# DonsetPG/graph-physics

Hardware: AMD Instinct MI355X
Metric: training steps/sec, CylinderFlow 15-round MGN (batch 16 meshes per step) (higher is better)
Workload: dtype f32; 1 GPU; BASELINE.json configs[1], fp32: 16 x 1885-node CylinderFlow-like meshes per GPU (N=30160, E=180082), 15 rounds, latent 128, random init; global_batch_meshes=16, launch=eager, parallelism=single

## Files before the change

### graph-physics_amd/csrc/mgn_kernels.hip

```cpp
#include <hip/hip_runtime.h>
#include <stdint.h>
#include <stdlib.h>
#include <type_traits>
#include "mgn_hip.h"

typedef float f32x4 __attribute__((ext_vector_type(4)));

#define MFMA16(a, b, c) __builtin_amdgcn_mfma_f32_16x16x4f32((a), (b), (c), 0, 0, 0)

typedef __attribute__((address_space(1))) const f32x4 g_cf32x4;
typedef __attribute__((address_space(1))) f32x4 g_f32x4;
typedef __attribute__((address_space(1))) const float g_cfloat;
typedef __attribute__((address_space(1))) float g_float;
__device__ __forceinline__ f32x4 ld4(const float* p) { return *(g_cf32x4*)p; }
__device__ __forceinline__ void st4(float* p, f32x4 v) { *(g_f32x4*)p = v; }
__device__ __forceinline__ void st4_stream(float* p, f32x4 v) { *(g_f32x4*)p = v; }
__device__ __forceinline__ float ld1(const float* p) { return *(g_cfloat*)p; }
__device__ __forceinline__ void st1(float* p, float v) { *(g_float*)p = v; }

template <int HB, int MT>
__device__ __forceinline__ void gemm_tl(f32x4 (&acc)[MT][HB], const f32x4 (&in)[MT][HB],
                                        const float* __restrict__ W, int ldw, int nib, int nkb,
                                        int c, int g) {
  const float* wl = W + (size_t)c * ldw + 4 * g;
  constexpr int IP = (HB >= 2) ? 2 : 1;
#pragma unroll
  for (int ib = 0; ib < HB; ib += IP) {
    if (ib < nib) {
#pragma unroll
      for (int kb = 0; kb < HB; ++kb) {
        if (kb < nkb) {
          f32x4 w[IP];
#pragma unroll
          for (int q = 0; q < IP; ++q)
            w[q] = (ib + q < nib) ? ld4(wl + (size_t)(16 * (ib + q)) * ldw + 16 * kb) : f32x4{0.f, 0.f, 0.f, 0.f};
#pragma unroll
          for (int r = 0; r < 4; ++r)
#pragma unroll
            for (int t = 0; t < MT; ++t)
#pragma unroll
              for (int q = 0; q < IP; ++q)
                acc[t][ib + q] = MFMA16(w[q][r], in[t][kb][r], acc[t][ib + q]);
        }
      }
    }
  }
}

template <int HB, int MT, bool NEXT>
__device__ __forceinline__ void gemm_full(f32x4 (&acc)[MT][HB], f32x4 (&in)[MT][HB],
                                          const float* __restrict__ W, int ldw, int c, int g,
                                          const float* const (&nxt)[MT]) {
  constexpr int IP = (HB >= 2) ? 2 : 1;
  constexpr int NI = HB / IP;
  constexpr int NS = HB * NI;
// ... 1295 lines not shown
    const unsigned nb0 = sm0 + (buf ^ 1) * 2 * WG_TILE_BYTES;
    lds_char* ta = sm + buf * 2 * WG_TILE_BYTES;
    lds_char* tb = ta + WG_TILE_BYTES;
    const bool tail = (tile + 1) * WG_TILE_ROWS > J.M;
    float av[2][8], bv[2][2];
    ld_quad(ta, tb, 0, av[0], bv[0]);
    const int rows_left = (int)(J.M - tile * WG_TILE_ROWS);
    auto body = [&](auto TAIL) {
#pragma unroll
      for (int quad = 0; quad < WG_TILE_ROWS / 4; ++quad) {
        if (quad + 1 < WG_TILE_ROWS / 4) ld_quad(ta, tb, quad + 1, av[(quad + 1) & 1], bv[(quad + 1) & 1]);
        if (more && quad < 4) {
          dma_row_piece(J.A, (tile + 1) * WG_TILE_ROWS, J.M, nb0, wv, lane, quad);
          dma_row_piece(J.B, (tile + 1) * WG_TILE_ROWS, J.M, nb0 + WG_TILE_BYTES, wv, lane, quad);
        }
        __builtin_amdgcn_sched_barrier(0);
        if (decltype(TAIL)::value) {
          const float keep = (4 * quad + g < rows_left) ? 1.f : 0.f;
#pragma unroll
          for (int jb = 0; jb < 8; ++jb) av[quad & 1][jb] *= keep;
        }
#pragma unroll
        for (int kk = 0; kk < 2; ++kk)
#pragma unroll
          for (int jb = 0; jb < 8; ++jb) acc[kk][jb] = MFMA16(av[quad & 1][jb], bv[quad & 1][kk], acc[kk][jb]);
        if (want_db) {
#pragma unroll
          for (int jb = 0; jb < 8; ++jb) cs[jb] += av[quad & 1][jb];
        }
        __builtin_amdgcn_sched_barrier(0);
      }
    };
    if (tail)
      body(std::true_type{});
    else
      body(std::false_type{});
    TL_STAMP(7);
  }
  TL_DUMP();
  float* P = L.partial + (size_t)blockIdx.x * (128 * 128 + 128);
  if (want_db) {
#pragma unroll
    for (int jb = 0; jb < 8; ++jb) {
      const float v = rowsum4(cs[jb]);
      if (g == 0) P[128 * 128 + 16 * jb + c] = v;
    }
  }
#pragma unroll
  for (int kk = 0; kk < 2; ++kk)
#pragma unroll
    for (int jb = 0; jb < 8; ++jb)
#pragma unroll
      for (int q = 0; q < 4; ++q) P[(16 * jb + 4 * g + q) * 128 + 16 * (kb0 + kk) + c] = acc[kk][jb][q];
}

#include "mgn_x6.inc"
#include "mgn_pp.inc"
#include "mgn_ppr.inc"
#include "mgn_fused.inc"

template <bool BF, bool A16 = false, bool B16 = false>
__global__ void __launch_bounds__(256, 2) k_wgrad_row64(const WgradLaunch L) {
  constexpr int H = 64;
  __shared__ float red[3][H * H + H];
  const int lane = threadIdx.x & 63, wv = threadIdx.x >> 6;
  const int c = lane & 15, g = lane >> 4;
  int j, wg, nwg;
  wgrad_where(L, j, wg, nwg);
  const mgn_wgrad_job J = L.job[j];
  const int pidx = L.wg0[j] + wg;
  const long ntiles = (J.M + 15) >> 4;
  const long t0 = ntiles * wg / nwg, t1 = ntiles * (wg + 1) / nwg;
  const bool a_on = 4 * c < 16 * J.nja, b_on = 4 * c < J.kw;

  f32x4 acc[4][4];
#pragma unroll
  for (int qa = 0; qa < 4; ++qa)
#pragma unroll
    for (int qb = 0; qb < 4; ++qb) acc[qa][qb] = f32x4{0.f, 0.f, 0.f, 0.f};
  f32x4 cs = {0.f, 0.f, 0.f, 0.f};
  const f32x4 zero = {0.f, 0.f, 0.f, 0.f};
  f32x4 av[2][4], bv[2][4];
  constexpr bool a16 = BF && A16, b16 = BF && B16;
  const long plda = A16 ? -(long)J.lda : J.lda, pldb = B16 ? -(long)J.ldb : J.ldb;
  auto ld16 = [&](const float* X, long off) -> f32x4 {
    const uint2 t = *(const uint2*)((const uint16_t*)X + off);
    return f32x4{__uint_as_float(t.x << 16), __uint_as_float(t.x & 0xffff0000u), __uint_as_float(t.y << 16), __uint_as_float(t.y & 0xffff0000u)};
  };
  auto load_tile = [&](long tile, f32x4 (&a)[4], f32x4 (&b)[4]) {
#pragma unroll
    for (int r = 0; r < 4; ++r) {
      const long row = tile * 16 + 4 * g + r;
      const bool ok = row < J.M;
      if constexpr (a16) a[r] = (ok && a_on) ? ld16(J.A, row * plda + 4 * c) : zero;
      else a[r] = (ok && a_on) ? ld4(J.A + row * plda + 4 * c) : zero;
      if constexpr (b16) b[r] = (ok && b_on) ? ld16(J.B, row * pldb + 4 * c) : zero;
      else b[r] = (ok && b_on) ? ld4(J.B + row * pldb + 4 * c) : zero;
    }
  };
  auto mac_tile = [&](const f32x4 (&a)[4], const f32x4 (&b)[4]) {
    if constexpr (BF) {
      typedef short s16x4 __attribute__((ext_vector_type(4)));
      typedef u32 u32x2_ __attribute__((ext_vector_type(2)));
      s16x4 pa[4], pb[4];
#pragma unroll
      for (int q = 0; q < 4; ++q) {
// ... 1104 lines not shown
    case 128: lrc = launch_bwd<8>(a, s); break;
    case 64: lrc = launch_bwd<4>(a, s); break;
    case 32: lrc = launch_bwd<2>(a, s); break;
    default: lrc = launch_bwd<1>(a, s); break;
  }
  if (lrc) return fail(2, "mgn_mlp_bwd: cannot reserve LDS");
  if (int rc = check_launch("mgn_mlp_bwd")) return rc;
  const unsigned grid = plan_mlp(a.M, a.H, a.NL, a.out_w != a.H || a.n_din > 1, true, a.act).grid;
  const int nslot = a.NL + 1;
  ColredOuts outs;
  bool any = false;
  for (int l = 0; l <= MGN_MAX_LAYERS; ++l) outs.o[l] = nullptr;
  for (int l = 0; l < a.NL; ++l) {
    outs.o[l] = a.db[l];
    any |= a.db[l] != nullptr;
  }
  outs.o[a.NL] = (a.scale != nullptr) ? a.dscale : nullptr;
  any |= outs.o[a.NL] != nullptr;
  if (!any || a.defer_reduce) return 0;
  const int n = nslot * a.H;
  hipLaunchKernelGGL(k_colred, dim3((n + 31) / 32), dim3(1024), 0, s, (const float*)a.red_ws, (int)grid, nslot, a.H, outs);
  return check_launch("mgn_mlp_bwd/colred");
}

int mgn_colred_batch(int n, const mgn_colred_job* jobs, void* stream) {
  if (n < 0) return fail(1, "mgn_colred_batch: bad arguments");
  hipStream_t s = (hipStream_t)stream;
  for (int i0 = 0; i0 < n; i0 += CR_MAX) {
    ColredBatch B;
    const int m = (n - i0 < CR_MAX) ? n - i0 : CR_MAX;
    int maxcol = 0;
    for (int i = 0; i < m; ++i) {
      const mgn_colred_job& q = jobs[i0 + i];
      if (q.red_ws == nullptr || q.NL < 1 || q.NL > MGN_MAX_LAYERS) return fail(1, "mgn_colred_batch: bad job");
      ColredJob& J = B.j[i];
      J.ws = (const float*)q.red_ws;
      J.nblocks = (int)plan_mlp(q.M, q.H, q.NL, q.out_w != q.H || q.n_din > 1, true).grid;
      J.nslot = q.NL + 1;
      J.H = q.H;
      for (int l = 0; l <= MGN_MAX_LAYERS; ++l) J.outs.o[l] = nullptr;
      for (int l = 0; l < q.NL; ++l) J.outs.o[l] = q.db[l];
      J.outs.o[q.NL] = q.dscale;
      if (J.nslot * J.H > maxcol) maxcol = J.nslot * J.H;
    }
    hipLaunchKernelGGL(k_colred_batch, dim3((maxcol + 31) / 32, m), dim3(1024), 0, s, B);
  }
  return check_launch("mgn_colred_batch");
}

static bool wgrad_job_row64(const mgn_wgrad_job& j) {
  return j.nja <= 4 && j.nkb <= 4 && j.kw <= 64 && (j.kw & 3) == 0 && (j.lda & 3) == 0 && (j.ldb & 3) == 0 &&
         (((uintptr_t)j.A | (uintptr_t)j.B) & 15) == 0;
}
static int wgrad_plan(int njobs, const mgn_wgrad_job* jobs, int* wg0, bool lds, int lds_budget = 512) {
  const int rows = lds ? WG_TILE_ROWS : 16;
  int budget = lds ? lds_budget : 512;
  if (!lds) {
    if (const char* e = getenv("MGN_WGRAD_GENERIC_BUDGET")) {
      const int b = atoi(e);
      if (b >= 64 && b <= 1024) budget = b;
    }
  }
  int64_t tiles[MGN_MAX_WGRAD_JOBS], tot = 0;
  int n[MGN_MAX_WGRAD_JOBS];
  for (int j = 0; j < njobs; ++j) {
    tiles[j] = (jobs[j].M + rows - 1) / rows;
    if (tiles[j] < 1) tiles[j] = 1;
    tot += tiles[j];
  }
  int used = 0;
  for (int j = 0; j < njobs; ++j) {
    int64_t s = tiles[j] * budget / tot;
    const int64_t cap = (tiles[j] + 3) / 4;
    if (s > cap) s = cap;
    if (s < 1) s = 1;
    n[j] = (int)s;
    used += n[j];
  }
  while (used < budget) {
    int best = -1;
    double load = 4.0;
    for (int j = 0; j < njobs; ++j) {
      const double l = (double)tiles[j] / n[j];
      if (l > load) {
        load = l;
        best = j;
      }
    }
    if (best < 0) break;
    ++n[best];
    ++used;
  }
  int acc = 0;
  for (int j = 0; j < njobs; ++j) {
    wg0[j] = acc;
    acc += n[j];
  }
  wg0[njobs] = acc;
  return acc;
}

size_t mgn_wgrad_workspace_bytes(int njobs, const mgn_wgrad_job* jobs) {
  if (njobs < 1 || njobs > MGN_MAX_WGRAD_JOBS) return 0;
  return (size_t)(512 + 1024 + 2 * MGN_MAX_WGRAD_JOBS) * (128 * 128 + 128) * sizeof(float);
}

static bool wgrad_job_full(const mgn_wgrad_job& j) {
  return j.nja == 8 && j.nkb == 8 && (j.lda == 128 || j.lda == -128) && (j.ldb == 128 || j.ldb == -128) && j.kw == 128 && j.M >= 1 && getenv("MGN_NO_LDS") == nullptr;
}

int mgn_wgrad(int njobs, const mgn_wgrad_job* jobs, void* ws, size_t ws_bytes, void* stream) {
  return mgn_wgrad_p(njobs, jobs, ws, ws_bytes, 0, stream);
}

int mgn_wgrad_p(int njobs, const mgn_wgrad_job* jobs, void* ws, size_t ws_bytes, int precision, void* stream) {
  if (precision != 0 && precision != 1) return fail(1, "mgn_wgrad: precision must be 0 (fp32-grade) or 1 (bf16)");
  if (njobs < 1 || njobs > MGN_MAX_WGRAD_JOBS) return fail(1, "mgn_wgrad: njobs out of range");
  for (int j = 0; j < njobs; ++j) {
    if (jobs[j].lda < 0 || jobs[j].ldb < 0) {
      const bool r64 = !wgrad_job_full(jobs[j]) && wgrad_job_row64(jobs[j]) && getenv("MGN_WGRAD_NO_ROW64") == nullptr &&
                       ((((uintptr_t)jobs[j].A | (uintptr_t)jobs[j].B) & 15) == 0);
      if (precision != 1 || !(wgrad_job_full(jobs[j]) || r64) || getenv("MGN_FP32_MFMA") != nullptr)
        return fail(1, "mgn_wgrad: a negative leading dimension (bf16 rows) needs precision 1 and a full 128 x 128 job with ld = -128 or a job of the row-vector kernel");
    }
  }
  hipStream_t s = (hipStream_t)stream;
  size_t ws_off = 0;
  for (int pass = 0; pass < 2; ++pass) {
    WgradLaunch L;
    L.njobs = 0;
    int maxb = 1;
    for (int j = 0; j < njobs; ++j) {
      if (jobs[j].nja < 1 || jobs[j].nkb < 1 || jobs[j].nja > 8 || jobs[j].nkb > 8) return fail(1, "mgn_wgrad: block counts out of range");
      if (wgrad_job_full(jobs[j]) != (pass == 0)) continue;
      L.job[L.njobs++] = jobs[j];
      if (jobs[j].nja > maxb) maxb = jobs[j].nja;
      if (jobs[j].nkb > maxb) maxb = jobs[j].nkb;
    }
    if (L.njobs == 0) continue;
    int HB = maxb <= 1 ? 1 : maxb <= 2 ? 2 : maxb <= 4 ? 4 : 8;
    bool row64 = pass == 1 && HB <= 4 && getenv("MGN_WGRAD_NO_ROW64") == nullptr;
    for (int j = 0; row64 && j < L.njobs; ++j) row64 = wgrad_job_row64(L.job[j]);
    if (row64) HB = 4;
    if (!row64 && pass == 1)
      for (int j = 0; j < L.njobs; ++j)
        if (L.job[j].lda < 0 || L.job[j].ldb < 0) return fail(1, "mgn_wgrad: bf16-row jobs below 128 x 128 need every job of the launch on the row-vector kernel");
    L.H = 16 * HB;
    bool pc = pass == 0 && precision == 0 && getenv("MGN_FP32_MFMA") == nullptr;
    if (pc) {
      const char* e = getenv("MGN_WGRAD_PC");
      pc = e == nullptr || atoi(e) != 0;
      for (int j = 0; pc && j < L.njobs; ++j) pc = L.job[j].lda == 128 && L.job[j].ldb == 128;
    }
    int total = wgrad_plan(L.njobs, L.job, L.wg0, pass == 0, pc ? 256 : 512);
    L.interleave = 0;
    if (row64 && L.njobs >= 2 && L.njobs <= 8 && getenv("MGN_WGRAD_NO_INTERLEAVE") == nullptr) {
      bool same = true;
      for (int j = 1; j < L.njobs; ++j) same = same && L.job[j].M == L.job[0].M;
      const int64_t tiles = (L.job[0].M + 15) / 16;
      int per = (512 / L.njobs) & ~7;
      while (per > 8 && (int64_t)per * 4 > tiles) per -= 8;
      if (same && per >= 8 && tiles >= 4 * per) {
        for (int j = 0; j <= L.njobs; ++j) L.wg0[j] = j * per;
        L.interleave = per;
        total = L.njobs * per;
      }
    }
    const size_t need = (size_t)total * (L.H * L.H + L.H) * sizeof(float);
    if (ws_bytes < ws_off + need) return fail(1, "mgn_wgrad: workspace too small");
    L.partial = (float*)((char*)ws + ws_off);
    ws_off += need;
    if (pc) {
      static thread_local bool attr_pc_done = false;
      if (!attr_pc_done) {
        if (hipFuncSetAttribute((const void*)k_wgrad_pc, hipFuncAttributeMaxDynamicSharedMemorySize, WPC_LDS_BYTES) != hipSuccess)
          return fail(2, "mgn_wgrad: cannot reserve LDS");
        attr_pc_done = true;
      }
      hipLaunchKernelGGL(k_wgrad_pc, dim3(total), dim3(512), WPC_LDS_BYTES, s, L);
    } else if (pass == 0) {
      const size_t smem = 4 * WG_TILE_BYTES;
      static thread_local bool attr_done = false;
      if (!attr_done) {
        if (hipFuncSetAttribute((const void*)k_wgrad_lds, hipFuncAttributeMaxDynamicSharedMemorySize, (int)smem) != hipSuccess)
          return fail(2, "mgn_wgrad: cannot reserve LDS");
        attr_done = true;
      }
      if (getenv("MGN_FP32_MFMA") == nullptr) {
        static thread_local bool attr6_done = false;
        if (!attr6_done) {
          if (hipFuncSetAttribute((const void*)k_wgrad_x6<6>, hipFuncAttributeMaxDynamicSharedMemorySize, (int)smem) != hipSuccess ||
              hipFuncSetAttribute((const void*)k_wgrad_x6<1>, hipFuncAttributeMaxDynamicSharedMemorySize, (int)smem) != hipSuccess)
            return fail(2, "mgn_wgrad: cannot reserve LDS");
          attr6_done = true;
        }
        if (precision == 1)
          hipLaunchKernelGGL(k_wgrad_x6<1>, dim3(total), dim3(256), smem, s, L);
        else
          hipLaunchKernelGGL(k_wgrad_x6<6>, dim3(total), dim3(256), smem, s, L);
      } else {
        hipLaunchKernelGGL(k_wgrad_lds, dim3(total), dim3(256), smem, s, L);
      }
    } else if (row64) {
      if (precision == 1) {
        const bool a16 = L.job[0].lda < 0, b16 = L.job[0].ldb < 0;
        for (int j = 1; j < L.njobs; ++j)
          if ((L.job[j].lda < 0) != a16 || (L.job[j].ldb < 0) != b16) return fail(1, "mgn_wgrad: the jobs of a row-vector launch must agree on which operand is bf16 rows");
        if (a16 && b16) hipLaunchKernelGGL((k_wgrad_row64<true, true, true>), dim3(total), dim3(256), 0, s, L);
        else if (a16) hipLaunchKernelGGL((k_wgrad_row64<true, true, false>), dim3(total), dim3(256), 0, s, L);
        else if (b16) hipLaunchKernelGGL((k_wgrad_row64<true, false, true>), dim3(total), dim3(256), 0, s, L);
        else hipLaunchKernelGGL((k_wgrad_row64<true>), dim3(total), dim3(256), 0, s, L);
      }
      else if (getenv("MGN_FP32_MFMA") == nullptr && getenv("MGN_WGRAD_ROW64_EXACT") == nullptr) {
        bool full = true;
        for (int j = 0; full && j < L.njobs; ++j) full = L.job[j].nja == 4 && L.job[j].kw == 64;
        if (full)
          hipLaunchKernelGGL(k_wgrad_row64x6<true>, dim3(total), dim3(256), 0, s, L);
        else
          hipLaunchKernelGGL(k_wgrad_row64x6<false>, dim3(total), dim3(256), 0, s, L);
      }
      else
        hipLaunchKernelGGL(k_wgrad_row64<false>, dim3(total), dim3(256), 0, s, L);
    } else {
      switch (HB) {
        case 8: hipLaunchKernelGGL(k_wgrad<8>, dim3(total), dim3(256), 0, s, L); break;
        case 4: hipLaunchKernelGGL(k_wgrad<4>, dim3(total), dim3(256), 0, s, L); break;
        case 2: hipLaunchKernelGGL(k_wgrad<2>, dim3(total), dim3(256), 0, s, L); break;
        default: hipLaunchKernelGGL(k_wgrad<1>, dim3(total), dim3(256), 0, s, L); break;
      }
    }
    if (int rc = check_launch("mgn_wgrad")) return rc;
    int max_nwg = 0;
    for (int j = 0; j < L.njobs; ++j) max_nwg = (L.wg0[j + 1] - L.wg0[j] > max_nwg) ? L.wg0[j + 1] - L.wg0[j] : max_nwg;
    if (max_nwg <= 64)
      hipLaunchKernelGGL(k_wgrad_red<4>, dim3((L.H * L.H + L.H + 63) / 64, L.njobs), dim3(64 * 4), 0, s, L);
    else
      hipLaunchKernelGGL(k_wgrad_red<16>, dim3((L.H * L.H + L.H + 63) / 64, L.njobs), dim3(64 * 16), 0, s, L);
    if (int rc = check_launch("mgn_wgrad/reduce")) return rc;
  }
  return 0;
}

int mgn_debug_occupancy(int* out) {
  int n = 0;
  if (hipFuncSetAttribute((const void*)k_mlp_fwd_x6<6, 4, 0>, hipFuncAttributeMaxDynamicSharedMemorySize, X6_FWD_LDS_BYTES(4)) != hipSuccess) return 1;
  if (hipFuncSetAttribute((const void*)k_mlp_fwd_x6<1, 4, 0>, hipFuncAttributeMaxDynamicSharedMemorySize, X6_FWD_LDS_BYTES(4)) != hipSuccess) return 1;
  if (hipFuncSetAttribute((const void*)k_mlp_fwd_x6<6, 8, 0>, hipFuncAttributeMaxDynamicSharedMemorySize, X6_FWD_LDS_BYTES(8)) != hipSuccess) return 1;
  if (hipFuncSetAttribute((const void*)k_mlp_bwd_x6<6, false, 0>, hipFuncAttributeMaxDynamicSharedMemorySize, X6_BWD_LDS_BYTES(LDS_MAX_NL + 1)) != hipSuccess) return 1;
// ... 47 lines not shown
```

### graph-physics_amd/csrc/mgn_x6.inc

```

typedef unsigned u32;
typedef u32 u32x4 __attribute__((ext_vector_type(4)));
typedef u32 u32x2 __attribute__((ext_vector_type(2)));
typedef __bf16 bf16x8 __attribute__((ext_vector_type(8)));
typedef __attribute__((address_space(3))) const u32x4 lds_cu32x4;

#define X6_QBYTES 24576
#define X6_RING 3
#define X6_FWD_LDS_BYTES(NW) (((NW) == 8 ? 6 : 3) * X6_QBYTES + 5 * 512)
#define X6_MAX_UNITS 8

#define MFMA_BF(a, b, c) \
  __builtin_amdgcn_mfma_f32_16x16x32_bf16(__builtin_bit_cast(bf16x8, (a)), __builtin_bit_cast(bf16x8, (b)), (c), 0, 0, 0)

typedef float f32x2 __attribute__((ext_vector_type(2)));
typedef __bf16 bf16x2 __attribute__((ext_vector_type(2)));
__device__ __forceinline__ u32 pk_bf16(float a, float b) {
  const f32x2 v = {a, b};
  return __builtin_bit_cast(u32, __builtin_convertvector(v, bf16x2));
}
__device__ __forceinline__ float bf_lo(u32 q) { return __builtin_bit_cast(float, q << 16); }
__device__ __forceinline__ float bf_hi(u32 q) { return __builtin_bit_cast(float, q & 0xffff0000u); }

__device__ __forceinline__ void split2(float a, float b, u32& q1, u32& q2, u32& q3) {
// ... 1324 lines not shown
        if (is_a) {
          if (rows_left < WG_TILE_ROWS) {
#pragma unroll
            for (int h = 0; h < 4; ++h) {
              const int r0_ = 8 * g + 2 * h;
              w[h] = (r0_ >= rows_left) ? 0u : ((r0_ + 1 >= rows_left) ? (w[h] & 0xffffu) : w[h]);
            }
          }
          if (want_db) cs[o] += ((bf_lo(w[0]) + bf_hi(w[0])) + (bf_lo(w[1]) + bf_hi(w[1]))) + ((bf_lo(w[2]) + bf_hi(w[2])) + (bf_lo(w[3]) + bf_hi(w[3])));
        }
        out[o][0] = w, out[o][1] = w, out[o][2] = w;
      }
    };
    if (a16) {
      take16(ta, jb0, true, ap);
    } else {
      take(ta, jb0, true, ap, 0);
      take(ta, jb0, true, ap, 2);
    }
    if (b16) {
      take16(tb, kb0, false, bp);
    } else {
      take(tb, kb0, false, bp, 0);
      take(tb, kb0, false, bp, 2);
    }
#pragma unroll
    for (int term = (TERMS == 1 ? 5 : 0); term < 6; ++term) {
      const int pa = (term == 0) ? 2 : (term == 1) ? 0 : (term == 2 || term == 3) ? 1 : 0;
      const int pb = (term == 0) ? 0 : (term == 1) ? 2 : (term == 2) ? 1 : (term == 3) ? 0 : (term == 4) ? 1 : 0;
#pragma unroll
      for (int jj = 0; jj < 4; ++jj)
#pragma unroll
        for (int kk = 0; kk < 4; ++kk) acc[jj][kk] = MFMA_BF(ap[jj][pa], bp[kk][pb], acc[jj][kk]);
    }
  }
  float* P = L.partial + (size_t)blockIdx.x * (128 * 128 + 128);
  if (want_db) {
#pragma unroll
    for (int jj = 0; jj < 4; ++jj) {
      const float v = rowsum4(cs[jj]);
      if (g == 0) P[128 * 128 + 16 * (jb0 + jj) + c] = v;
    }
  }
#pragma unroll
  for (int jj = 0; jj < 4; ++jj)
#pragma unroll
    for (int kk = 0; kk < 4; ++kk)
#pragma unroll
      for (int q = 0; q < 4; ++q) P[(16 * (jb0 + jj) + 4 * g + q) * 128 + 16 * (kb0 + kk) + c] = acc[jj][kk][q];
}

#define WPC_IMG 49152
#define WPC_NIMG 3
#define WPC_LDS_BYTES (WPC_NIMG * WPC_IMG + 64)
#ifdef MGN_TIMELINE
__device__ unsigned long long g_wpc_tl[2][2048];
__device__ int g_wpc_tln[2];
__device__ unsigned long long g_wpc_wg[512][2];
#define WPC_TL_DECL()                                   \
  int tl_n_ = 0;                                        \
  const bool tl_on_ = blockIdx.x == 0 && (threadIdx.x == 0 || threadIdx.x == 256)
#define WPC_STAMP(tag)                                                                                                  \
  do {                                                                                                                  \
    if (tl_on_ && tl_n_ < 2048) g_wpc_tl[threadIdx.x >> 8][tl_n_++] = (__builtin_readcyclecounter() << 8) | (tag);      \
  } while (0)
#define WPC_TL_DUMP()                               \
  do {                                              \
    WPC_STAMP(9);                                   \
    if (tl_on_ && tl_n_ < 2048) g_wpc_tl[threadIdx.x >> 8][tl_n_++] = (__builtin_amdgcn_s_memrealtime() << 8) | 8; \
    if (tl_on_) g_wpc_tln[threadIdx.x >> 8] = tl_n_; \
  } while (0)
extern "C" int mgn_debug_wpc_wgtimes(unsigned long long* out) {
  return hipMemcpyFromSymbol(out, HIP_SYMBOL(g_wpc_wg), sizeof(unsigned long long) * 512 * 2) != hipSuccess;
}
extern "C" int mgn_debug_wpc_timeline(unsigned long long* out, int* n) {
  if (hipMemcpyFromSymbol(out, HIP_SYMBOL(g_wpc_tl), sizeof(unsigned long long) * 2 * 2048) != hipSuccess) return 1;
  return hipMemcpyFromSymbol(n, HIP_SYMBOL(g_wpc_tln), sizeof(int) * 2) != hipSuccess;
}
#else
#define WPC_TL_DECL() ((void)0)
#define WPC_STAMP(tag) ((void)0)
#define WPC_TL_DUMP() ((void)0)
#endif
__device__ __forceinline__ void wpc_barrier() {
  asm volatile("s_waitcnt lgkmcnt(0)" ::: "memory");
  __builtin_amdgcn_sched_barrier(0);
  __builtin_amdgcn_s_barrier();
  __builtin_amdgcn_sched_barrier(0);
  asm volatile("" ::: "memory");
}
__device__ __forceinline__ void wpc_barrier_c() {
  __builtin_amdgcn_sched_barrier(0);
  __builtin_amdgcn_s_barrier();
  __builtin_amdgcn_sched_barrier(0);
}

__global__ void __launch_bounds__(512, 2) k_wgrad_pc(const WgradLaunch L) {
  extern __shared__ __attribute__((aligned(16))) char smem[];
  lds_char* sm = (lds_char*)smem;
  const int lane = threadIdx.x & 63;
  const int wv = __builtin_amdgcn_readfirstlane(threadIdx.x >> 6);
  int j = 0;
  while (j + 1 < L.njobs && (int)blockIdx.x >= L.wg0[j + 1]) ++j;
  const mgn_wgrad_job J = L.job[j];
  const int nwg = L.wg0[j + 1] - L.wg0[j];
  const int wg = blockIdx.x - L.wg0[j];
  const long ntiles = (J.M + WG_TILE_ROWS - 1) / WG_TILE_ROWS;
  const long t0 = 0, t1 = (ntiles - wg + nwg - 1) / nwg;
  auto gtile = [&](long k) { return (long)wg + k * nwg; };
  const bool has_last = t1 > 0 && gtile(t1 - 1) == ntiles - 1;
  float* P = L.partial + (size_t)blockIdx.x * (128 * 128 + 128);
  WPC_TL_DECL();
#ifdef MGN_TIMELINE
  if (tl_on_) g_wpc_tl[threadIdx.x >> 8][tl_n_++] = (__builtin_amdgcn_s_memrealtime() << 8) | 8;
  WPC_STAMP(7);
  if (threadIdx.x == 0 && blockIdx.x < 512) g_wpc_wg[blockIdx.x][0] = __builtin_amdgcn_s_memrealtime();
#endif

  if (wv < 4) {
    __builtin_amdgcn_s_setprio(1);
    const int mat = wv >> 1, half = wv & 1;
    const int rg = lane >> 5, q = lane & 31;
    const int g = 2 * half + rg;
    const float* X = mat ? J.B : J.A;
    const int b = q >> 2;
    const int s = (((q >> 1) & 1) << 1) | (b & 1);
    lds_char* wa[4];
#pragma unroll
    for (int e = 0; e < 4; ++e) wa[e] = sm + ((mat * 8 + b) * 3) * 1024 + g * 256 + 64 * (q & 3) + 16 * (e ^ s);
    const bool want_db = (mat == 0) && (J.db != nullptr);
    f32x4 cs = {0.f, 0.f, 0.f, 0.f};
    f32x4 raw0[8], raw1[8], raw2[8], raw3[8];
    const WgSel wsel = wg_sel(lane & 15, lane >> 4);
    const long tf = (has_last && (J.M % WG_TILE_ROWS) != 0) ? t1 - 1 : t1;
    auto load_tile = [&](long tile_, f32x4 (&raw)[8]) {
      const long kk = tile_ < tf ? tile_ : tf - 1;
      const long tile = gtile(kk);
      const float* p = X + (tile * WG_TILE_ROWS + 8 * g) * 128 + 4 * q;
#pragma unroll
      for (int i = 0; i < 8; ++i) raw[i] = ld4(p + i * 128);
    };
    auto process = [&](f32x4 (&raw)[8], int buf) {
      if (want_db) {
#pragma unroll
        for (int e = 0; e < 4; ++e)
          cs[e] += ((raw[0][e] + raw[1][e]) + (raw[2][e] + raw[3][e])) + ((raw[4][e] + raw[5][e]) + (raw[6][e] + raw[7][e]));
      }
      WPC_STAMP(1);
      typedef __attribute__((address_space(3))) u32x4 lds_u32x4;
      f32x4 r0[4], r1[4];
      u32x4 p1[4], p2[4], p3[4];
#pragma unroll
      for (int e = 0; e < 4; ++e) {
        r0[e] = f32x4{raw[0][e], raw[1][e], raw[2][e], raw[3][e]};
        r1[e] = f32x4{raw[4][e], raw[5][e], raw[6][e], raw[7][e]};
        p1[e] = u32x4{pk_bf16(raw[0][e], raw[1][e]), pk_bf16(raw[2][e], raw[3][e]), pk_bf16(raw[4][e], raw[5][e]), pk_bf16(raw[6][e], raw[7][e])};
      }
      __builtin_amdgcn_sched_barrier(0);
#pragma unroll
      for (int e = 0; e < 4; ++e) r0[e] = MFMA_BF(wsel.s0, p1[e], r0[e]), r1[e] = MFMA_BF(wsel.s1, p1[e], r1[e]);
      __builtin_amdgcn_sched_barrier(0);
#pragma unroll
      for (int e = 0; e < 4; ++e) {
        lds_char* d = wa[e] + buf;
        *(lds_u32x4*)(d) = p1[e];
        p2[e] = u32x4{pk_bf16(r0[e][0], r0[e][1]), pk_bf16(r0[e][2], r0[e][3]), pk_bf16(r1[e][0], r1[e][1]), pk_bf16(r1[e][2], r1[e][3])};
      }
      __builtin_amdgcn_sched_barrier(0);
#pragma unroll
      for (int e = 0; e < 4; ++e) r0[e] = MFMA_BF(wsel.s0, p2[e], r0[e]), r1[e] = MFMA_BF(wsel.s1, p2[e], r1[e]);
      __builtin_amdgcn_sched_barrier(0);
#pragma unroll
      for (int e = 0; e < 4; ++e) {
        lds_char* d = wa[e] + buf;
        *(lds_u32x4*)(d + 1024) = p2[e];
        p3[e] = u32x4{pk_bf16(r0[e][0], r0[e][1]), pk_bf16(r0[e][2], r0[e][3]), pk_bf16(r1[e][0], r1[e][1]), pk_bf16(r1[e][2], r1[e][3])};
        *(lds_u32x4*)(d + 2048) = p3[e];
      }
    };
    int img = 0;
    auto next_img = [&]() { img = (img == (WPC_NIMG - 1) * WPC_IMG) ? 0 : img + WPC_IMG; };
    if (t0 < tf) {
      load_tile(t0, raw0);
      __builtin_amdgcn_sched_barrier(0);
      load_tile(t0 + 1, raw1);
      __builtin_amdgcn_sched_barrier(0);
      load_tile(t0 + 2, raw2);
      __builtin_amdgcn_sched_barrier(0);
      long tile = t0;
#define WPC_STEP(cur, nxt, ahead)            \
  WPC_STAMP(0);                              \
  load_tile(tile + ahead, nxt);              \
  __builtin_amdgcn_sched_barrier(0);         \
  WPC_STAMP(3);                              \
  process(cur, img);                         \
  WPC_STAMP(2);                              \
  next_img();                                \
  wpc_barrier()
      for (; tile + 3 < tf; tile += 4) {
        WPC_STEP(raw0, raw3, 3);
        WPC_STEP(raw1, raw0, 4);
        WPC_STEP(raw2, raw1, 5);
        WPC_STEP(raw3, raw2, 6);
      }
      if (tile < tf) {
        process(raw0, img);
        next_img();
        wpc_barrier();
      }
      if (tile + 1 < tf) {
        process(raw1, img);
        next_img();
        wpc_barrier();
      }
      if (tile + 2 < tf) {
        process(raw2, img);
        next_img();
        wpc_barrier();
      }
    }
    if (tf < t1) {
      const long r0 = gtile(tf) * WG_TILE_ROWS + 8 * g;
#pragma unroll
      for (int i = 0; i < 8; ++i) {
        long r = r0 + i;
        r = r < J.M ? r : J.M - 1;
        raw0[i] = ld4(X + r * 128 + 4 * q);
      }
      if (mat == 0) {
#pragma unroll
        for (int i = 0; i < 8; ++i)
          if (r0 + i >= J.M) raw0[i] = f32x4{0.f, 0.f, 0.f, 0.f};
      }
      process(raw0, img);
      wpc_barrier();
    }
    wpc_barrier();
    if (mat == 0) {
      typedef __attribute__((address_space(3))) f32x4 lds_f32x4;
      *(lds_f32x4*)(sm + (g * 128 + 4 * q) * 4) = cs;
    }
    wpc_barrier();
    if (want_db && wv == 0) {
      typedef __attribute__((address_space(3))) const float lds_cfloat;
#pragma unroll
      for (int h = 0; h < 2; ++h) {
        const int f = lane + 64 * h;
        lds_cfloat* r = (lds_cfloat*)sm + f;
        P[128 * 128 + f] = (r[0] + r[128]) + (r[256] + r[384]);
      }
    }
  } else {
    const int cw = wv - 4;
    const int c = lane & 15, g = lane >> 4;
    const int jb0 = 4 * (cw >> 1), kb0 = 4 * (cw & 1);
    f32x4 acc[4][4];
#pragma unroll
    for (int jj = 0; jj < 4; ++jj)
#pragma unroll
      for (int kk = 0; kk < 4; ++kk) acc[jj][kk] = f32x4{0.f, 0.f, 0.f, 0.f};
    const int sl0 = c ^ ((c >> 3) << 1);
    lds_char* ra[2] = {sm + (jb0 * 3) * 1024 + g * 256 + 16 * sl0, sm + (jb0 * 3) * 1024 + g * 256 + 16 * (sl0 ^ 1)};
    lds_char* rb[2] = {sm + ((8 + kb0) * 3) * 1024 + g * 256 + 16 * sl0, sm + ((8 + kb0) * 3) * 1024 + g * 256 + 16 * (sl0 ^ 1)};
    u32x4 ap[4][3], bp[4][3];
    auto rdA = [&](int p, int img) {
#pragma unroll
      for (int jj = 0; jj < 4; ++jj) ap[jj][p] = *(lds_cu32x4*)(ra[jj & 1] + img + jj * 3072 + p * 1024);
    };
    auto rdB = [&](int p, int img) {
#pragma unroll
      for (int kk = 0; kk < 4; ++kk) bp[kk][p] = *(lds_cu32x4*)(rb[kk & 1] + img + kk * 3072 + p * 1024);
    };
    auto term = [&](int pa, int pb) {
#pragma unroll
      for (int jj = 0; jj < 4; ++jj)
#pragma unroll
        for (int kk = 0; kk < 4; ++kk) acc[jj][kk] = MFMA_BF(ap[jj][pa], bp[kk][pb], acc[jj][kk]);
    };
    const long n = t1 - t0;
    if (n > 0) {
      wpc_barrier_c();
      rdA(0, 0), rdB(2, 0), rdB(1, 0), rdA(1, 0), rdB(0, 0), rdA(2, 0);
      int img = 0;
      for (long k = 1; k < n; ++k) {
        img = (img == (WPC_NIMG - 1) * WPC_IMG) ? 0 : img + WPC_IMG;
        WPC_STAMP(1);
        wpc_barrier_c();
        WPC_STAMP(0);
#define WPC_PIN() __builtin_amdgcn_sched_barrier(0)
        term(0, 2);
        WPC_PIN();
        rdB(2, img);
        WPC_PIN();
        term(0, 1);
        term(1, 1);
        WPC_PIN();
        rdB(1, img);
        WPC_PIN();
        term(0, 0);
        WPC_PIN();
        rdA(0, img);
        WPC_PIN();
        term(1, 0);
        WPC_PIN();
        rdA(1, img);
        WPC_PIN();
        term(2, 0);
        WPC_PIN();
        rdA(2, img);
        rdB(0, img);
      }
      term(0, 2);
      term(0, 1), term(1, 1), term(0, 0), term(1, 0);
      term(2, 0);
    }
    wpc_barrier();
    wpc_barrier();
#pragma unroll
    for (int jj = 0; jj < 4; ++jj)
#pragma unroll
      for (int kk = 0; kk < 4; ++kk)
#pragma unroll
        for (int qq = 0; qq < 4; ++qq) P[(16 * (jb0 + jj) + 4 * g + qq) * 128 + 16 * (kb0 + kk) + c] = acc[jj][kk][qq];
  }
  WPC_TL_DUMP();
#ifdef MGN_TIMELINE
  if (threadIdx.x == 0 && blockIdx.x < 512) g_wpc_wg[blockIdx.x][1] = __builtin_amdgcn_s_memrealtime();
#endif
}
```

Before: 83.06 steps/s.

## Split wgrad_pc tile range contiguously across workgroups spanning multiple jobs

Replaces the per-job workgroup budget of the packed-bf16 weight-gradient kernel with a global contiguous partition of all jobs' tiles over at most 256 workgroups. Each workgroup can now handle segments of several jobs in sequence, writing a separate partial slot per segment, and workgroups fully inside a job stride-interleave its tiles. The column-sum scratch moves to a dedicated LDS region so it no longer aliases the tile images. The aim is better load balance and fewer idle or short-lived workgroups. In exchange it adds per-segment barriers and epilogue writes, plus a more complex planner. LDS-attribute caching also becomes per-device and atomic.

```diff
diff --git a/graph-physics_amd/csrc/mgn_kernels.hip b/graph-physics_amd/csrc/mgn_kernels.hip
--- a/graph-physics_amd/csrc/mgn_kernels.hip
+++ b/graph-physics_amd/csrc/mgn_kernels.hip
@@ -1,6 +1,9 @@
 #include <hip/hip_runtime.h>
 #include <stdint.h>
 #include <stdlib.h>
+#include <string.h>
+#include <algorithm>
+#include <atomic>
 #include <type_traits>
 #include "mgn_hip.h"
 
@@ -1402,6 +1405,49 @@
     for (int jb = 0; jb < 8; ++jb)
 #pragma unroll
       for (int q = 0; q < 4; ++q) P[(16 * jb + 4 * g + q) * 128 + 16 * (kb0 + kk) + c] = acc[kk][jb][q];
+}
+
+#define WPC_MAX_WG 256
+#define WPC_SEGMENT_TILES 3
+struct WpcJob {
+  const float* A;
+  const float* B;
+  int64_t M;
+  int64_t want_db;
+};
+struct WpcLaunch {
+  WpcJob job[MGN_MAX_WGRAD_JOBS];
+  float* partial;
+  int njobs, nwg;
+  int s[WPC_MAX_WG + 1];
+  int g0[MGN_MAX_WGRAD_JOBS];
+  unsigned short wa[MGN_MAX_WGRAD_JOBS];
+  unsigned short wf[MGN_MAX_WGRAD_JOBS], nfull[MGN_MAX_WGRAD_JOBS];
+  unsigned short slot0[MGN_MAX_WGRAD_JOBS];
+};
+static_assert(sizeof(WpcLaunch) <= 4096, "kernel arguments: 4 KB");
+struct WpcSeg {
+  int first, count, stride;
+  int slot;
+};
+__host__ __device__ inline WpcSeg wpc_segment(const WpcLaunch& L, int w, int j) {
+  WpcSeg S;
+  const int g = L.g0[j], gend = g + (int)((L.job[j].M + WG_TILE_ROWS - 1) / WG_TILE_ROWS);
+  const int wf = L.wf[j], nf = L.nfull[j];
+  const bool alone = w >= wf && w < wf + nf;
+  const int a = alone ? L.s[wf] : L.s[w], b = alone ? L.s[wf + nf] : L.s[w + 1];
+  const int lo = (a > g ? a : g) - g, hi = (b < gend ? b : gend) - g;
+  if (alone) {
+    S.first = lo + (w - wf);
+    S.stride = nf;
+    S.count = (hi - S.first + nf - 1) / nf;
+  } else {
+    S.first = lo;
+    S.stride = 1;
+    S.count = hi - lo;
+  }
+  S.slot = (int)L.slot0[j] + (w - (int)L.wa[j]);
+  return S;
 }
 
 #include "mgn_x6.inc"
@@ -2612,9 +2658,19 @@
   return j.nja <= 4 && j.nkb <= 4 && j.kw <= 64 && (j.kw & 3) == 0 && (j.lda & 3) == 0 && (j.ldb & 3) == 0 &&
          (((uintptr_t)j.A | (uintptr_t)j.B) & 15) == 0;
 }
-static int wgrad_plan(int njobs, const mgn_wgrad_job* jobs, int* wg0, bool lds, int lds_budget = 512) {
+static bool reserve_lds(const void* fn, int bytes, std::atomic<uint64_t>& done) {
+  int dev = 0;
+  if (hipGetDevice(&dev) != hipSuccess) return false;
+  const uint64_t bit = dev < 64 ? (uint64_t)1 << dev : 0;
+  if (done.load(std::memory_order_relaxed) & bit) return true;
+  if (hipFuncSetAttribute(fn, hipFuncAttributeMaxDynamicSharedMemorySize, bytes) != hipSuccess) return false;
+  done.fetch_or(bit, std::memory_order_relaxed);
+  return true;
+}
+
+static int wgrad_plan(int njobs, const mgn_wgrad_job* jobs, int* wg0, bool lds) {
   const int rows = lds ? WG_TILE_ROWS : 16;
-  int budget = lds ? lds_budget : 512;
+  int budget = 512;
   if (!lds) {
     if (const char* e = getenv("MGN_WGRAD_GENERIC_BUDGET")) {
       const int b = atoi(e);
@@ -2660,8 +2716,71 @@
   return acc;
 }
 
+static int wpc_plan(int njobs, const mgn_wgrad_job* jobs, WpcLaunch& P, int* slot_of_job) {
+  int64_t tot = 0, len = 0;
+  int64_t tiles[MGN_MAX_WGRAD_JOBS];
+  for (int j = 0; j < njobs; ++j) {
+    tiles[j] = (jobs[j].M + WG_TILE_ROWS - 1) / WG_TILE_ROWS;
+    tot += tiles[j];
+  }
+  const int nwg = (int)std::min<int64_t>(WPC_MAX_WG, std::max<int64_t>(1, (tot + 3) / 4));
+  const int64_t gap = std::min<int64_t>(WPC_SEGMENT_TILES, tot / nwg / 4);
+  for (int j = 0; j < njobs; ++j) {
+    if (j > 0) len += gap;
+    if (len + tiles[j] >= INT32_MAX) return -1;
+    P.job[j] = WpcJob{jobs[j].A, jobs[j].B, jobs[j].M, jobs[j].db != nullptr};
+    P.g0[j] = (int)len;
+    len += tiles[j];
+  }
+  P.njobs = njobs;
+  P.nwg = nwg;
+  for (int w = 0; w <= nwg; ++w) P.s[w] = (int)(len * w / nwg);
+  int first[MGN_MAX_WGRAD_JOBS], last[MGN_MAX_WGRAD_JOBS], w = 0, slots = 0;
+  for (int j = 0; j < njobs; ++j) {
+    const int g = P.g0[j], gend = g + (int)tiles[j];
+    while (P.s[w + 1] <= g) ++w;
+    first[j] = w;
+    while (P.s[w + 1] < gend) ++w;
+    last[j] = w;
+  }
+  for (int j = 0; j < njobs; ++j) {
+    const bool shares_first = j > 0 && last[j - 1] == first[j], shares_last = j + 1 < njobs && first[j + 1] == last[j];
+    const int wf = first[j] + (shares_first ? 1 : 0), wl = last[j] - (shares_last ? 1 : 0);
+    P.wa[j] = (unsigned short)first[j];
+    P.wf[j] = (unsigned short)wf;
+    P.nfull[j] = (unsigned short)(wl >= wf ? wl - wf + 1 : 0);
+    P.slot0[j] = (unsigned short)slots;
+    slot_of_job[j] = slots;
+    slots += last[j] - first[j] + 1;
+  }
+  slot_of_job[njobs] = slots;
+  return slots;
+}
+
+extern "C" int mgn_debug_wgrad_segments(int njobs, const mgn_wgrad_job* jobs, int* out, int cap) {
+  if (njobs < 1 || njobs > MGN_MAX_WGRAD_JOBS) return -1;
+  WpcLaunch P;
+  int slot_of_job[MGN_MAX_WGRAD_JOBS + 1];
+  for (int j = 0; j < njobs; ++j)
+    if (jobs[j].M < 1) return -1;
+  if (wpc_plan(njobs, jobs, P, slot_of_job) < 0) return -1;
+  int n = 0;
+  for (int w = 0; w < P.nwg; ++w)
+    for (int j = 0; j < njobs; ++j) {
+      const WpcSeg S = wpc_segment(P, w, j);
+      if (S.count <= 0) continue;
+      if (n < cap) {
+        const int row[6] = {w, j, S.first, S.count, S.stride, S.slot};
+        memcpy(out + 6 * n, row, sizeof(row));
+      }
+      ++n;
+    }
+  return n <= cap ? n : -1;
+}
+
 size_t mgn_wgrad_workspace_bytes(int njobs, const mgn_wgrad_job* jobs) {
   if (njobs < 1 || njobs > MGN_MAX_WGRAD_JOBS) return 0;
+  static_assert(WPC_MAX_WG <= 512, "k_wgrad_pc's slots fit the full jobs' share of the workspace");
   return (size_t)(512 + 1024 + 2 * MGN_MAX_WGRAD_JOBS) * (128 * 128 + 128) * sizeof(float);
 }
 
@@ -2712,7 +2831,9 @@
       pc = e == nullptr || atoi(e) != 0;
       for (int j = 0; pc && j < L.njobs; ++j) pc = L.job[j].lda == 128 && L.job[j].ldb == 128;
     }
-    int total = wgrad_plan(L.njobs, L.job, L.wg0, pass == 0, pc ? 256 : 512);
+    WpcLaunch P;
+    int total = pc ? wpc_plan(L.njobs, L.job, P, L.wg0) : wgrad_plan(L.njobs, L.job, L.wg0, pass == 0);
+    if (total < 0) return fail(1, "mgn_wgrad: too many rows for one launch");
     L.interleave = 0;
     if (row64 && L.njobs >= 2 && L.njobs <= 8 && getenv("MGN_WGRAD_NO_INTERLEAVE") == nullptr) {
       bool same = true;
@@ -2731,29 +2852,17 @@
     L.partial = (float*)((char*)ws + ws_off);
     ws_off += need;
     if (pc) {
-      static thread_local bool attr_pc_done = false;
-      if (!attr_pc_done) {
-        if (hipFuncSetAttribute((const void*)k_wgrad_pc, hipFuncAttributeMaxDynamicSharedMemorySize, WPC_LDS_BYTES) != hipSuccess)
-          return fail(2, "mgn_wgrad: cannot reserve LDS");
-        attr_pc_done = true;
-      }
-      hipLaunchKernelGGL(k_wgrad_pc, dim3(total), dim3(512), WPC_LDS_BYTES, s, L);
+      static std::atomic<uint64_t> attr_pc_done{0};
+      if (!reserve_lds((const void*)k_wgrad_pc, WPC_LDS_BYTES, attr_pc_done)) return fail(2, "mgn_wgrad: cannot reserve LDS");
+      P.partial = L.partial;
+      hipLaunchKernelGGL(k_wgrad_pc, dim3(P.nwg), dim3(512), WPC_LDS_BYTES, s, P);
     } else if (pass == 0) {
       const size_t smem = 4 * WG_TILE_BYTES;
-      static thread_local bool attr_done = false;
-      if (!attr_done) {
-        if (hipFuncSetAttribute((const void*)k_wgrad_lds, hipFuncAttributeMaxDynamicSharedMemorySize, (int)smem) != hipSuccess)
+      static std::atomic<uint64_t> attr_done{0}, attr6_done{0}, attr1_done{0};
+      if (!reserve_lds((const void*)k_wgrad_lds, (int)smem, attr_done)) return fail(2, "mgn_wgrad: cannot reserve LDS");
+      if (getenv("MGN_FP32_MFMA") == nullptr) {
+        if (!reserve_lds((const void*)k_wgrad_x6<6>, (int)smem, attr6_done) || !reserve_lds((const void*)k_wgrad_x6<1>, (int)smem, attr1_done))
           return fail(2, "mgn_wgrad: cannot reserve LDS");
-        attr_done = true;
-      }
-      if (getenv("MGN_FP32_MFMA") == nullptr) {
-        static thread_local bool attr6_done = false;
-        if (!attr6_done) {
-          if (hipFuncSetAttribute((const void*)k_wgrad_x6<6>, hipFuncAttributeMaxDynamicSharedMemorySize, (int)smem) != hipSuccess ||
-              hipFuncSetAttribute((const void*)k_wgrad_x6<1>, hipFuncAttributeMaxDynamicSharedMemorySize, (int)smem) != hipSuccess)
-            return fail(2, "mgn_wgrad: cannot reserve LDS");
-          attr6_done = true;
-        }
         if (precision == 1)
           hipLaunchKernelGGL(k_wgrad_x6<1>, dim3(total), dim3(256), smem, s, L);
         else
diff --git a/graph-physics_amd/csrc/mgn_x6.inc b/graph-physics_amd/csrc/mgn_x6.inc
--- a/graph-physics_amd/csrc/mgn_x6.inc
+++ b/graph-physics_amd/csrc/mgn_x6.inc
@@ -1400,7 +1400,8 @@
 
 #define WPC_IMG 49152
 #define WPC_NIMG 3
-#define WPC_LDS_BYTES (WPC_NIMG * WPC_IMG + 64)
+#define WPC_DB_BYTES 2048
+#define WPC_LDS_BYTES (WPC_NIMG * WPC_IMG + WPC_DB_BYTES + 64)
 #ifdef MGN_TIMELINE
 __device__ unsigned long long g_wpc_tl[2][2048];
 __device__ int g_wpc_tln[2];
@@ -1443,21 +1444,15 @@
   __builtin_amdgcn_sched_barrier(0);
 }
 
-__global__ void __launch_bounds__(512, 2) k_wgrad_pc(const WgradLaunch L) {
+__global__ void __launch_bounds__(512, 2) k_wgrad_pc(const WpcLaunch L) {
   extern __shared__ __attribute__((aligned(16))) char smem[];
   lds_char* sm = (lds_char*)smem;
   const int lane = threadIdx.x & 63;
   const int wv = __builtin_amdgcn_readfirstlane(threadIdx.x >> 6);
+  const int w = blockIdx.x;
+  const int s_lo = L.s[w], s_hi = L.s[w + 1];
   int j = 0;
-  while (j + 1 < L.njobs && (int)blockIdx.x >= L.wg0[j + 1]) ++j;
-  const mgn_wgrad_job J = L.job[j];
-  const int nwg = L.wg0[j + 1] - L.wg0[j];
-  const int wg = blockIdx.x - L.wg0[j];
-  const long ntiles = (J.M + WG_TILE_ROWS - 1) / WG_TILE_ROWS;
-  const long t0 = 0, t1 = (ntiles - wg + nwg - 1) / nwg;
-  auto gtile = [&](long k) { return (long)wg + k * nwg; };
-  const bool has_last = t1 > 0 && gtile(t1 - 1) == ntiles - 1;
-  float* P = L.partial + (size_t)blockIdx.x * (128 * 128 + 128);
+  while (j + 1 < L.njobs && L.g0[j + 1] <= s_lo) ++j;
   WPC_TL_DECL();
 #ifdef MGN_TIMELINE
   if (tl_on_) g_wpc_tl[threadIdx.x >> 8][tl_n_++] = (__builtin_amdgcn_s_memrealtime() << 8) | 8;
@@ -1470,72 +1465,81 @@
     const int mat = wv >> 1, half = wv & 1;
     const int rg = lane >> 5, q = lane & 31;
     const int g = 2 * half + rg;
-    const float* X = mat ? J.B : J.A;
     const int b = q >> 2;
     const int s = (((q >> 1) & 1) << 1) | (b & 1);
     lds_char* wa[4];
 #pragma unroll
     for (int e = 0; e < 4; ++e) wa[e] = sm + ((mat * 8 + b) * 3) * 1024 + g * 256 + 64 * (q & 3) + 16 * (e ^ s);
-    const bool want_db = (mat == 0) && (J.db != nullptr);
-    f32x4 cs = {0.f, 0.f, 0.f, 0.f};
     f32x4 raw0[8], raw1[8], raw2[8], raw3[8];
     const WgSel wsel = wg_sel(lane & 15, lane >> 4);
-    const long tf = (has_last && (J.M % WG_TILE_ROWS) != 0) ? t1 - 1 : t1;
-    auto load_tile = [&](long tile_, f32x4 (&raw)[8]) {
-      const long kk = tile_ < tf ? tile_ : tf - 1;
-      const long tile = gtile(kk);
-      const float* p = X + (tile * WG_TILE_ROWS + 8 * g) * 128 + 4 * q;
-#pragma unroll
-      for (int i = 0; i < 8; ++i) raw[i] = ld4(p + i * 128);
-    };
-    auto process = [&](f32x4 (&raw)[8], int buf) {
-      if (want_db) {
-#pragma unroll
-        for (int e = 0; e < 4; ++e)
-          cs[e] += ((raw[0][e] + raw[1][e]) + (raw[2][e] + raw[3][e])) + ((raw[4][e] + raw[5][e]) + (raw[6][e] + raw[7][e]));
-      }
-      WPC_STAMP(1);
-      typedef __attribute__((address_space(3))) u32x4 lds_u32x4;
-      f32x4 r0[4], r1[4];
-      u32x4 p1[4], p2[4], p3[4];
-#pragma unroll
-      for (int e = 0; e < 4; ++e) {
-        r0[e] = f32x4{raw[0][e], raw[1][e], raw[2][e], raw[3][e]};
-        r1[e] = f32x4{raw[4][e], raw[5][e], raw[6][e], raw[7][e]};
-        p1[e] = u32x4{pk_bf16(raw[0][e], raw[1][e]), pk_bf16(raw[2][e], raw[3][e]), pk_bf16(raw[4][e], raw[5][e]), pk_bf16(raw[6][e], raw[7][e])};
-      }
-      __builtin_amdgcn_sched_barrier(0);
-#pragma unroll
-      for (int e = 0; e < 4; ++e) r0[e] = MFMA_BF(wsel.s0, p1[e], r0[e]), r1[e] = MFMA_BF(wsel.s1, p1[e], r1[e]);
-      __builtin_amdgcn_sched_barrier(0);
-#pragma unroll
-      for (int e = 0; e < 4; ++e) {
-        lds_char* d = wa[e] + buf;
-        *(lds_u32x4*)(d) = p1[e];
-        p2[e] = u32x4{pk_bf16(r0[e][0], r0[e][1]), pk_bf16(r0[e][2], r0[e][3]), pk_bf16(r1[e][0], r1[e][1]), pk_bf16(r1[e][2], r1[e][3])};
-      }
-      __builtin_amdgcn_sched_barrier(0);
-#pragma unroll
-      for (int e = 0; e < 4; ++e) r0[e] = MFMA_BF(wsel.s0, p2[e], r0[e]), r1[e] = MFMA_BF(wsel.s1, p2[e], r1[e]);
-      __builtin_amdgcn_sched_barrier(0);
-#pragma unroll
-      for (int e = 0; e < 4; ++e) {
-        lds_char* d = wa[e] + buf;
-        *(lds_u32x4*)(d + 1024) = p2[e];
-        p3[e] = u32x4{pk_bf16(r0[e][0], r0[e][1]), pk_bf16(r0[e][2], r0[e][3]), pk_bf16(r1[e][0], r1[e][1]), pk_bf16(r1[e][2], r1[e][3])};
-        *(lds_u32x4*)(d + 2048) = p3[e];
-      }
-    };
-    int img = 0;
-    auto next_img = [&]() { img = (img == (WPC_NIMG - 1) * WPC_IMG) ? 0 : img + WPC_IMG; };
-    if (t0 < tf) {
-      load_tile(t0, raw0);
-      __builtin_amdgcn_sched_barrier(0);
-      load_tile(t0 + 1, raw1);
-      __builtin_amdgcn_sched_barrier(0);
-      load_tile(t0 + 2, raw2);
-      __builtin_amdgcn_sched_barrier(0);
-      long tile = t0;
+    for (; j < L.njobs && L.g0[j] < s_hi; ++j) {
+      const WpcSeg S = wpc_segment(L, w, j);
+      if (S.count <= 0) continue;
+      const WpcJob J = L.job[j];
+      const long ntiles = (J.M + WG_TILE_ROWS - 1) / WG_TILE_ROWS;
+      const long t0 = 0, t1 = S.count;
+      auto gtile = [&](long k) { return (long)S.first + k * S.stride; };
+      const bool has_last = gtile(t1 - 1) == ntiles - 1;
+      float* P = L.partial + (size_t)S.slot * (128 * 128 + 128);
+      const float* X = mat ? J.B : J.A;
+      const bool want_db = (mat == 0) && (J.want_db != 0);
+      f32x4 cs = {0.f, 0.f, 0.f, 0.f};
+      const long tf = (has_last && (J.M % WG_TILE_ROWS) != 0) ? t1 - 1 : t1;
+      auto load_tile = [&](long tile_, f32x4 (&raw)[8]) {
+        const long kk = tile_ < tf ? tile_ : tf - 1;
+        const long tile = gtile(kk);
+        const float* p = X + (tile * WG_TILE_ROWS + 8 * g) * 128 + 4 * q;
+#pragma unroll
+        for (int i = 0; i < 8; ++i) raw[i] = ld4(p + i * 128);
+      };
+      auto process = [&](f32x4 (&raw)[8], int buf) {
+        if (want_db) {
+#pragma unroll
+          for (int e = 0; e < 4; ++e)
+            cs[e] += ((raw[0][e] + raw[1][e]) + (raw[2][e] + raw[3][e])) + ((raw[4][e] + raw[5][e]) + (raw[6][e] + raw[7][e]));
+        }
+        WPC_STAMP(1);
+        typedef __attribute__((address_space(3))) u32x4 lds_u32x4;
+        f32x4 r0[4], r1[4];
+        u32x4 p1[4], p2[4], p3[4];
+#pragma unroll
+        for (int e = 0; e < 4; ++e) {
+          r0[e] = f32x4{raw[0][e], raw[1][e], raw[2][e], raw[3][e]};
+          r1[e] = f32x4{raw[4][e], raw[5][e], raw[6][e], raw[7][e]};
+          p1[e] = u32x4{pk_bf16(raw[0][e], raw[1][e]), pk_bf16(raw[2][e], raw[3][e]), pk_bf16(raw[4][e], raw[5][e]), pk_bf16(raw[6][e], raw[7][e])};
+        }
+        __builtin_amdgcn_sched_barrier(0);
+#pragma unroll
+        for (int e = 0; e < 4; ++e) r0[e] = MFMA_BF(wsel.s0, p1[e], r0[e]), r1[e] = MFMA_BF(wsel.s1, p1[e], r1[e]);
+        __builtin_amdgcn_sched_barrier(0);
+#pragma unroll
+        for (int e = 0; e < 4; ++e) {
+          lds_char* d = wa[e] + buf;
+          *(lds_u32x4*)(d) = p1[e];
+          p2[e] = u32x4{pk_bf16(r0[e][0], r0[e][1]), pk_bf16(r0[e][2], r0[e][3]), pk_bf16(r1[e][0], r1[e][1]), pk_bf16(r1[e][2], r1[e][3])};
+        }
+        __builtin_amdgcn_sched_barrier(0);
+#pragma unroll
+        for (int e = 0; e < 4; ++e) r0[e] = MFMA_BF(wsel.s0, p2[e], r0[e]), r1[e] = MFMA_BF(wsel.s1, p2[e], r1[e]);
+        __builtin_amdgcn_sched_barrier(0);
+#pragma unroll
+        for (int e = 0; e < 4; ++e) {
+          lds_char* d = wa[e] + buf;
+          *(lds_u32x4*)(d + 1024) = p2[e];
+          p3[e] = u32x4{pk_bf16(r0[e][0], r0[e][1]), pk_bf16(r0[e][2], r0[e][3]), pk_bf16(r1[e][0], r1[e][1]), pk_bf16(r1[e][2], r1[e][3])};
+          *(lds_u32x4*)(d + 2048) = p3[e];
+        }
+      };
+      int img = 0;
+      auto next_img = [&]() { img = (img == (WPC_NIMG - 1) * WPC_IMG) ? 0 : img + WPC_IMG; };
+      if (t0 < tf) {
+        load_tile(t0, raw0);
+        __builtin_amdgcn_sched_barrier(0);
+        load_tile(t0 + 1, raw1);
+        __builtin_amdgcn_sched_barrier(0);
+        load_tile(t0 + 2, raw2);
+        __builtin_amdgcn_sched_barrier(0);
+        long tile = t0;
 #define WPC_STEP(cur, nxt, ahead)            \
   WPC_STAMP(0);                              \
   load_tile(tile + ahead, nxt);              \
@@ -1545,57 +1549,58 @@
   WPC_STAMP(2);                              \
   next_img();                                \
   wpc_barrier()
-      for (; tile + 3 < tf; tile += 4) {
-        WPC_STEP(raw0, raw3, 3);
-        WPC_STEP(raw1, raw0, 4);
-        WPC_STEP(raw2, raw1, 5);
-        WPC_STEP(raw3, raw2, 6);
-      }
-      if (tile < tf) {
+        for (; tile + 3 < tf; tile += 4) {
+          WPC_STEP(raw0, raw3, 3);
+          WPC_STEP(raw1, raw0, 4);
+          WPC_STEP(raw2, raw1, 5);
+          WPC_STEP(raw3, raw2, 6);
+        }
+        if (tile < tf) {
+          process(raw0, img);
+          next_img();
+          wpc_barrier();
+        }
+        if (tile + 1 < tf) {
+          process(raw1, img);
+          next_img();
+          wpc_barrier();
+        }
+        if (tile + 2 < tf) {
+          process(raw2, img);
+          next_img();
+          wpc_barrier();
+        }
+      }
+      if (tf < t1) {
+        const long r0 = gtile(tf) * WG_TILE_ROWS + 8 * g;
+#pragma unroll
+        for (int i = 0; i < 8; ++i) {
+          long r = r0 + i;
+          r = r < J.M ? r : J.M - 1;
+          raw0[i] = ld4(X + r * 128 + 4 * q);
+        }
+        if (mat == 0) {
+#pragma unroll
+          for (int i = 0; i < 8; ++i)
+            if (r0 + i >= J.M) raw0[i] = f32x4{0.f, 0.f, 0.f, 0.f};
+        }
         process(raw0, img);
-        next_img();
         wpc_barrier();
       }
-      if (tile + 1 < tf) {
-        process(raw1, img);
-        next_img();
-        wpc_barrier();
-      }
-      if (tile + 2 < tf) {
-        process(raw2, img);
-        next_img();
-        wpc_barrier();
-      }
-    }
-    if (tf < t1) {
-      const long r0 = gtile(tf) * WG_TILE_ROWS + 8 * g;
-#pragma unroll
-      for (int i = 0; i < 8; ++i) {
-        long r = r0 + i;
-        r = r < J.M ? r : J.M - 1;
-        raw0[i] = ld4(X + r * 128 + 4 * q);
-      }
+      wpc_barrier();
       if (mat == 0) {
-#pragma unroll
-        for (int i = 0; i < 8; ++i)
-          if (r0 + i >= J.M) raw0[i] = f32x4{0.f, 0.f, 0.f, 0.f};
-      }
-      process(raw0, img);
+        typedef __attribute__((address_space(3))) f32x4 lds_f32x4;
+        *(lds_f32x4*)(sm + WPC_NIMG * WPC_IMG + (g * 128 + 4 * q) * 4) = cs;
+      }
       wpc_barrier();
-    }
-    wpc_barrier();
-    if (mat == 0) {
-      typedef __attribute__((address_space(3))) f32x4 lds_f32x4;
-      *(lds_f32x4*)(sm + (g * 128 + 4 * q) * 4) = cs;
-    }
-    wpc_barrier();
-    if (want_db && wv == 0) {
-      typedef __attribute__((address_space(3))) const float lds_cfloat;
-#pragma unroll
-      for (int h = 0; h < 2; ++h) {
-        const int f = lane + 64 * h;
-        lds_cfloat* r = (lds_cfloat*)sm + f;
-        P[128 * 128 + f] = (r[0] + r[128]) + (r[256] + r[384]);
+      if (want_db && wv == 0) {
+        typedef __attribute__((address_space(3))) const float lds_cfloat;
+#pragma unroll
+        for (int h = 0; h < 2; ++h) {
+          const int f = lane + 64 * h;
+          lds_cfloat* r = (lds_cfloat*)(sm + WPC_NIMG * WPC_IMG) + f;
+          P[128 * 128 + f] = (r[0] + r[128]) + (r[256] + r[384]);
+        }
       }
     }
   } else {
@@ -1603,10 +1608,6 @@
     const int c = lane & 15, g = lane >> 4;
     const int jb0 = 4 * (cw >> 1), kb0 = 4 * (cw & 1);
     f32x4 acc[4][4];
-#pragma unroll
-    for (int jj = 0; jj < 4; ++jj)
-#pragma unroll
-      for (int kk = 0; kk < 4; ++kk) acc[jj][kk] = f32x4{0.f, 0.f, 0.f, 0.f};
     const int sl0 = c ^ ((c >> 3) << 1);
     lds_char* ra[2] = {sm + (jb0 * 3) * 1024 + g * 256 + 16 * sl0, sm + (jb0 * 3) * 1024 + g * 256 + 16 * (sl0 ^ 1)};
     lds_char* rb[2] = {sm + ((8 + kb0) * 3) * 1024 + g * 256 + 16 * sl0, sm + ((8 + kb0) * 3) * 1024 + g * 256 + 16 * (sl0 ^ 1)};
@@ -1625,51 +1626,60 @@
 #pragma unroll
         for (int kk = 0; kk < 4; ++kk) acc[jj][kk] = MFMA_BF(ap[jj][pa], bp[kk][pb], acc[jj][kk]);
     };
-    const long n = t1 - t0;
-    if (n > 0) {
-      wpc_barrier_c();
-      rdA(0, 0), rdB(2, 0), rdB(1, 0), rdA(1, 0), rdB(0, 0), rdA(2, 0);
-      int img = 0;
-      for (long k = 1; k < n; ++k) {
-        img = (img == (WPC_NIMG - 1) * WPC_IMG) ? 0 : img + WPC_IMG;
-        WPC_STAMP(1);
+    for (; j < L.njobs && L.g0[j] < s_hi; ++j) {
+      const WpcSeg S = wpc_segment(L, w, j);
+      if (S.count <= 0) continue;
+      float* P = L.partial + (size_t)S.slot * (128 * 128 + 128);
+#pragma unroll
+      for (int jj = 0; jj < 4; ++jj)
+#pragma unroll
+        for (int kk = 0; kk < 4; ++kk) acc[jj][kk] = f32x4{0.f, 0.f, 0.f, 0.f};
+      const long n = S.count;
+      {
         wpc_barrier_c();
-        WPC_STAMP(0);
+        rdA(0, 0), rdB(2, 0), rdB(1, 0), rdA(1, 0), rdB(0, 0), rdA(2, 0);
+        int img = 0;
+        for (long k = 1; k < n; ++k) {
+          img = (img == (WPC_NIMG - 1) * WPC_IMG) ? 0 : img + WPC_IMG;
+          WPC_STAMP(1);
+          wpc_barrier_c();
+          WPC_STAMP(0);
 #define WPC_PIN() __builtin_amdgcn_sched_barrier(0)
+          term(0, 2);
+          WPC_PIN();
+          rdB(2, img);
+          WPC_PIN();
+          term(0, 1);
+          term(1, 1);
+          WPC_PIN();
+          rdB(1, img);
+          WPC_PIN();
+          term(0, 0);
+          WPC_PIN();
+          rdA(0, img);
+          WPC_PIN();
+          term(1, 0);
+          WPC_PIN();
+          rdA(1, img);
+          WPC_PIN();
+          term(2, 0);
+          WPC_PIN();
+          rdA(2, img);
+          rdB(0, img);
+        }
         term(0, 2);
-        WPC_PIN();
-        rdB(2, img);
-        WPC_PIN();
-        term(0, 1);
-        term(1, 1);
-        WPC_PIN();
-        rdB(1, img);
-        WPC_PIN();
-        term(0, 0);
-        WPC_PIN();
-        rdA(0, img);
-        WPC_PIN();
-        term(1, 0);
-        WPC_PIN();
-        rdA(1, img);
-        WPC_PIN();
+        term(0, 1), term(1, 1), term(0, 0), term(1, 0);
         term(2, 0);
-        WPC_PIN();
-        rdA(2, img);
-        rdB(0, img);
-      }
-      term(0, 2);
-      term(0, 1), term(1, 1), term(0, 0), term(1, 0);
-      term(2, 0);
-    }
-    wpc_barrier();
-    wpc_barrier();
-#pragma unroll
-    for (int jj = 0; jj < 4; ++jj)
-#pragma unroll
-      for (int kk = 0; kk < 4; ++kk)
-#pragma unroll
-        for (int qq = 0; qq < 4; ++qq) P[(16 * (jb0 + jj) + 4 * g + qq) * 128 + 16 * (kb0 + kk) + c] = acc[jj][kk][qq];
+      }
+      wpc_barrier();
+      wpc_barrier();
+#pragma unroll
+      for (int jj = 0; jj < 4; ++jj)
+#pragma unroll
+        for (int kk = 0; kk < 4; ++kk)
+#pragma unroll
+          for (int qq = 0; qq < 4; ++qq) P[(16 * (jb0 + jj) + 4 * g + qq) * 128 + 16 * (kb0 + kk) + c] = acc[jj][kk][qq];
+    }
   }
   WPC_TL_DUMP();
 #ifdef MGN_TIMELINE
```

Result: no change. 82.82 steps/s (-0.3%).
